# yeyupiaoling/VoiceprintRecognition-Pytorch

Measured on NVIDIA H100. Metric: embeddings/sec (3s@16kHz) ECAPA-TDNN, higher is better.
Workload: dtype f32

## Files before the change

voiceprintrecognition-pytorch_b200/csrc/api.cu:

```cuda
#include <cmath>
#include <cstdarg>
#include <cstdio>
#include <cstdlib>
#include <cstring>
#include <new>
#include <string>
#include <vector>

#include "kernels.cuh"


using namespace vpb;

struct vp_handle {
  int device = 0;
  std::string err;
  float* d_weights = nullptr;
  size_t weights_bytes = 0;
  char* d_arena = nullptr;
  size_t arena_bytes = 0;
  cudaStream_t cap_stream = nullptr;
  bool fe_set = false;
  vp_frontend_desc fe{};
  vp_frontend_options fe_opt{VP_FRAME_DEFAULT, 0, 1.0};
  float* d_window = nullptr;
  double2* d_twiddle = nullptr;
  int* d_mel_start = nullptr;
  int* d_mel_count = nullptr;
  int* d_mel_off = nullptr;
  float* d_mel_w = nullptr;
  float* d_dct = nullptr;
};

struct vp_program {
  vp_handle* h = nullptr;
  std::vector<vp_op> ops;
  std::vector<int> engines;
  size_t ws_bytes = 0, in_floats = 0, out_floats = 0;
  int launches = 0;
  int B = 0;
  cudaGraphExec_t gexec = nullptr;
  const float* g_feats = nullptr;
  float* g_emb = nullptr;
  char* g_arena = nullptr;
  int runs = 0, g_miss = 0;
  bool g_off = false;
  int n_slots = 0;
  size_t arena_need() const { return ws_bytes + (((size_t)n_slots * 4 + 255) & ~(size_t)255); }
  unsigned* slot(int32_t q) const { return q > 0 ? reinterpret_cast<unsigned*>(h->d_arena + ws_bytes) + (q - 1) : nullptr; }
};

static int fail(vp_handle* h, int code, const char* fmt, ...) {
  char buf[512];
  va_list ap;
  va_start(ap, fmt);
  vsnprintf(buf, sizeof(buf), fmt, ap);
  va_end(ap);
  if (h) h->err = buf;
  return code;
}
#define CUDA_TRY(h, expr)                                                                          \
  do {                                                                                             \
    cudaError_t e__ = (expr);                                                                      \
    if (e__ != cudaSuccess) return fail(h, VP_ERR_CUDA, "%s: %s", #expr, cudaGetErrorString(e__)); \
  } while (0)

static const int FPB = 16;

static bool tc16_enabled() {
  static int on = -1;
  if (on < 0) { const char* e = getenv("VPB_TC_F16"); on = (e && e[0] == '0') ? 0 : 1; }
  return on == 1;
}

extern "C" {

static void fill_conv(const vp_program* p, const vp_op& o, const float* feats, float* emb, vpb::ConvParams& c);

int vp_abi_version(void) { return VP_ABI_VERSION; }
int32_t vp_sizeof_op(void) { return (int32_t)sizeof(vp_op); }
int32_t vp_sizeof_frontend_desc(void) { return (int32_t)sizeof(vp_frontend_desc); }
int32_t vp_sizeof_frontend_options(void) { return (int32_t)sizeof(vp_frontend_options); }

int vp_create(int device, vp_handle** out) {
  if (!out) return VP_ERR_INVALID;
  *out = nullptr;
  int n = 0;
  cudaError_t e = cudaGetDeviceCount(&n);
  if (e != cudaSuccess || device < 0 || device >= n) return VP_ERR_CUDA;
  cudaDeviceProp prop;
  if (cudaGetDeviceProperties(&prop, device) != cudaSuccess) return VP_ERR_CUDA;
  if (prop.major != 9 || prop.minor != 0) return VP_ERR_UNSUPPORTED;
  if (cudaSetDevice(device) != cudaSuccess) return VP_ERR_CUDA;
  vp_handle* h = new (std::nothrow) vp_handle();
  if (!h) return VP_ERR_NOMEM;
  h->device = device;
  *out = h;
  return VP_OK;
}

// ... 405 lines not shown
    ConvParams c;
    fill_conv(p, o, nullptr, nullptr, c);
    c.amax_in = o.amax_in > 0 ? reinterpret_cast<const unsigned*>(8) : nullptr;
    const bool ok = conv_tc_supported(c);
    bool ok16 = ok && o.w_tc16_q > 0 && o.tc16_descale > 0.f && conv_tc16_supported(c);
    if (ok16) {
      const int bn = o.tc_bn, nt = (o.Cout + bn - 1) / bn, kb = (c.K + 63) / 64;
      const size_t off = (size_t)(o.w_tc16_q - 1) << 4, bytes = (size_t)nt * kb * 2 * bn * 128;
      if (off + bytes > h->weights_bytes) {
        int r = fail(h, VP_ERR_INVALID, "op %d: fp16 weight image out of range", i);
        delete p;
        return r;
      }
    }
    if ((o.engine == VP_ENGINE_TC && !ok) || (o.engine == VP_ENGINE_TC16 && !ok16)) {
      int r = fail(h, VP_ERR_UNSUPPORTED, "op %d: shape / operands not supported by the requested tensor-core engine", i);
      delete p;
      return r;
    }
    if (o.engine == VP_ENGINE_TC16 || (o.engine == VP_ENGINE_AUTO && ok16 && tc16_enabled())) p->engines[i] = VP_ENGINE_TC16;
    else if (o.engine == VP_ENGINE_TC || (o.engine == VP_ENGINE_AUTO && ok)) p->engines[i] = VP_ENGINE_TC;
    else p->engines[i] = VP_ENGINE_FFMA;
  }
  if (cudaSetDevice(h->device) != cudaSuccess) { delete p; return fail(h, VP_ERR_CUDA, "cudaSetDevice"); }
  if (p->arena_need() > h->arena_bytes) {
    const size_t want = p->arena_need() + (p->arena_need() >> 3);
    cudaDeviceSynchronize();
    cudaFree(h->d_arena);
    h->d_arena = nullptr;
    h->arena_bytes = 0;
    if (cudaMalloc(&h->d_arena, want) != cudaSuccess) {
      cudaGetLastError();
      if (cudaMalloc(&h->d_arena, p->arena_need()) != cudaSuccess) {
        delete p;
        return fail(h, VP_ERR_NOMEM, "workspace of %zu bytes: %s", ws_bytes, cudaGetErrorString(cudaGetLastError()));
      }
      h->arena_bytes = p->arena_need();
    } else {
      h->arena_bytes = want;
    }
  }
  *out = p;
  return VP_OK;
}

void vp_program_destroy(vp_program* p) {
// ... 18 lines not shown

static void fill_conv(const vp_program* p, const vp_op& o, const float* feats, float* emb, ConvParams& c) {
  c.src = rd(p, o.src, feats, emb);
  c.src2 = o.src2_mode == VP_SRC2_NONE ? nullptr : rd(p, o.src2, feats, emb);
  c.dst = const_cast<float*>(rd(p, o.dst, feats, emb));
  c.sum = const_cast<float*>(rd(p, o.sum, feats, emb)); c.sum_ld = o.sum_ld; c.sum_coff = o.sum_coff;
  c.res = rd(p, o.res, feats, emb); c.gate = rd(p, o.gate, feats, emb); c.ubias = rd(p, o.ubias, feats, emb);
  c.w = wt(p, o.w); c.w_tc = wt(p, o.w_tc); c.tc_bn = o.tc_bn; c.tc_kc = o.tc_kc; c.bias = wt(p, o.bias); c.pre_s = wt(p, o.pre_s); c.pre_h = wt(p, o.pre_h);
  c.post_s = wt(p, o.post_s); c.post_h = wt(p, o.post_h);
  c.B = o.B; c.Tin = o.Tin; c.Fin = o.Fin; c.Cin = o.Cin;
  c.CinTot = o.Cin + (o.src2_mode == VP_SRC2_CONCAT ? o.Cin2 : 0);
  c.in_ld = o.in_ld; c.in_coff = o.in_coff;
  c.src2_mode = o.src2_mode; c.src2_ld = o.src2_ld; c.src2_coff = o.src2_coff;
  c.Tout = o.Tout; c.Fout = o.Fout; c.out_ld = o.out_ld; c.out_coff = o.out_coff;
  c.res_ld = o.res_ld; c.res_coff = o.res_coff;
  c.KT = o.KT; c.KF = o.KF; c.sT = o.sT; c.sF = o.sF; c.dT = o.dT; c.dF = o.dF; c.padT = o.padT; c.padF = o.padF;
  c.pad_mode = o.pad_mode; c.w_ld = o.w_ld; c.pre_relu = o.pre_relu; c.act = o.act; c.act2 = o.act2;
  c.seg_len = o.seg_len; c.n_seg = o.n_seg;
  c.M = o.B * o.Tout * o.Fout; c.N = o.Cout; c.K = o.KT * o.KF * c.CinTot;
  c.amax_out = p->h->d_arena ? p->slot(o.amax_out) : nullptr;
  c.amax_in = p->h->d_arena ? p->slot(o.amax_in) : nullptr;
}

static int run_ops(vp_program* p, const float* feats, float* emb, cudaStream_t st, cudaEvent_t* evs) {
  vp_handle* h = p->h;
  if (p->n_slots > 0) CUDA_TRY(h, cudaMemsetAsync(h->d_arena + p->ws_bytes, 0, (size_t)p->n_slots * 4, st));
  for (size_t i = 0; i < p->ops.size(); ++i) {
    const vp_op& o = p->ops[i];
    if (evs) CUDA_TRY(h, cudaEventRecord(evs[i], st));
    switch (o.kind) {
      case VP_OP_CONV:
      case VP_OP_CONV_C1: {
        ConvParams c;
        fill_conv(p, o, feats, emb, c);
        if (o.kind == VP_OP_CONV_C1) {
          CUDA_TRY(h, launch_conv_c1(c, st));
        } else {
          if (p->engines[i] == VP_ENGINE_TC16)
            CUDA_TRY(h, launch_conv_tc16(c, reinterpret_cast<const float*>(reinterpret_cast<const char*>(h->d_weights) + ((size_t)(o.w_tc16_q - 1) << 4)),
                                         o.tc16_descale, st));
          else if (p->engines[i] == VP_ENGINE_TC) CUDA_TRY(h, launch_conv_tc(c, st));
          else CUDA_TRY(h, launch_conv_ffma(c, st));
        }
        break;
      }
      case VP_OP_COLSTATS: {
        StatsParams s;
        s.src = rd(p, o.src, feats, emb); s.dst = const_cast<float*>(rd(p, o.dst, feats, emb));
        s.B = o.B; s.R = o.Tin * o.Fin; s.C = o.Cin; s.in_ld = o.in_ld; s.in_coff = o.in_coff;
        s.out_ld = o.out_ld; s.out_coff = o.out_coff; s.mode = o.mode; s.seg_len = o.seg_len; s.n_seg = o.n_seg;
        s.eps = o.eps;
        CUDA_TRY(h, launch_colstats(s, st));
        break;
      }
      case VP_OP_ASP_POOL: {
        AspParams a;
        a.x = rd(p, o.src, feats, emb); a.logit = rd(p, o.src2, feats, emb);
        a.dst = const_cast<float*>(rd(p, o.dst, feats, emb));
        a.B = o.B; a.T = o.Tin; a.C = o.Cin; a.x_ld = o.in_ld; a.x_coff = o.in_coff; a.l_ld = o.src2_ld;
        a.l_coff = o.src2_coff; a.out_ld = o.out_ld; a.out_coff = o.out_coff; a.eps = o.eps; a.mean_only = o.mode == 1;
        CUDA_TRY(h, launch_asp_pool(a, st));
        break;
      }
      case VP_OP_POOL2D: {
        PoolParams q;
        q.src = rd(p, o.src, feats, emb); q.dst = const_cast<float*>(rd(p, o.dst, feats, emb));
        q.B = o.B; q.Tin = o.Tin; q.Fin = o.Fin; q.Tout = o.Tout; q.Fout = o.Fout; q.C = o.Cin;
        q.in_ld = o.in_ld; q.in_coff = o.in_coff; q.out_ld = o.out_ld; q.out_coff = o.out_coff;
        q.KT = o.KT; q.KF = o.KF; q.sT = o.sT; q.sF = o.sF; q.padT = o.padT; q.padF = o.padF; q.mode = o.mode;
        q.amax_out = p->slot(o.amax_out);
        CUDA_TRY(h, launch_pool2d(q, st));
        break;
      }
      case VP_OP_EW: {
        EwParams e;
        e.x = rd(p, o.src, feats, emb);
        e.y = o.mode == VP_EW_AFF ? rd(p, o.src2, feats, emb) : nullptr;
        e.att = o.mode == VP_EW_AFF ? rd(p, o.res, feats, emb) : nullptr;
        e.gate = o.mode == VP_EW_GATE_RES ? rd(p, o.gate, feats, emb) : nullptr;
        e.res = o.mode == VP_EW_GATE_RES ? rd(p, o.res, feats, emb) : nullptr;
        e.dst = const_cast<float*>(rd(p, o.dst, feats, emb));
        e.rows = (long long)o.B * o.Tin * o.Fin; e.C = o.Cin; e.rows_per_utt = o.Tin * o.Fin;
        e.x_ld = o.in_ld; e.x_coff = o.in_coff; e.y_ld = o.src2_ld; e.y_coff = o.src2_coff;
        e.att_ld = o.res_ld; e.att_coff = o.res_coff; e.res_ld = o.res_ld; e.res_coff = o.res_coff;
// ... 223 lines not shown
```

voiceprintrecognition-pytorch_b200/csrc/conv_tc.cu:

```cuda
#include <cuda_fp16.h>

#include <cstdlib>
#include <type_traits>

#include "kernels.cuh"
#include "wgmma.cuh"

namespace vpb {

namespace tc {

constexpr int BM = 128;
constexpr int BK = 32;
constexpr int A_TILE = BM * BK * 4;
constexpr int CONSUMER_WARPS = 8;
constexpr int CONSUMER_THREADS = CONSUMER_WARPS * 32;
constexpr int PRODUCER_WARPS = 8;
constexpr int PRODUCER_THREADS = PRODUCER_WARPS * 32;
constexpr int NUM_THREADS = CONSUMER_THREADS + PRODUCER_THREADS;
constexpr int ROWS_PER_THREAD = BM * 8 / PRODUCER_THREADS;
constexpr int MAX_BN = 128;
constexpr int MAX_BN_CHUNKED = 64;
constexpr int SMEM_BUDGET = 225 * 1024;

__device__ __forceinline__ uint32_t smem_u32(const void* p) { return (uint32_t)__cvta_generic_to_shared(p); }

__device__ __forceinline__ void mbar_init(uint32_t bar, uint32_t count) {
  asm volatile("mbarrier.init.shared::cta.b64 [%0], %1;" ::"r"(bar), "r"(count));
}
__device__ __forceinline__ void mbar_arrive(uint32_t bar) {
  asm volatile("mbarrier.arrive.shared::cta.b64 _, [%0];" ::"r"(bar) : "memory");
}
__device__ __forceinline__ void mbar_expect_tx(uint32_t bar, uint32_t bytes) {
  asm volatile("mbarrier.arrive.expect_tx.shared::cta.b64 _, [%0], %1;" ::"r"(bar), "r"(bytes) : "memory");
}
__device__ __forceinline__ void mbar_wait(uint32_t bar, uint32_t parity) {
  asm volatile(
      "{\n\t.reg .pred p;\n\t"
      "WAIT_%=:\n\t"
      "mbarrier.try_wait.parity.shared::cta.b64 p, [%0], %1;\n\t"
      "@p bra DONE_%=;\n\t"
      "bra WAIT_%=;\n\t"
      "DONE_%=:\n\t}" ::"r"(bar), "r"(parity)
      : "memory");
}
__device__ __forceinline__ void bulk_copy_g2s(uint32_t dst, const void* src, uint32_t bytes, uint32_t bar) {
  asm volatile("cp.async.bulk.shared::cluster.global.mbarrier::complete_tx::bytes [%0], [%1], %2, [%3];" ::"r"(dst),
               "l"(src), "r"(bytes), "r"(bar)
               : "memory");
}
__device__ __forceinline__ void fence_proxy_async() { asm volatile("fence.proxy.async.shared::cta;" ::: "memory"); }

__device__ __forceinline__ void wgmma_fence() { asm volatile("wgmma.fence.sync.aligned;" ::: "memory"); }
__device__ __forceinline__ void wgmma_commit() { asm volatile("wgmma.commit_group.sync.aligned;" ::: "memory"); }
template <int N>
__device__ __forceinline__ void wgmma_wait() { asm volatile("wgmma.wait_group.sync.aligned %0;" ::"n"(N) : "memory"); }
template <int N>
__device__ __forceinline__ void fence_regs(float (&d)[N]) {
#pragma unroll
  for (int i = 0; i < N; ++i) asm volatile("" : "+f"(d[i])::"memory");
}

__device__ __forceinline__ uint64_t smem_desc(uint32_t addr) {
  return (uint64_t)((addr >> 4) & 0x3FFF) | (1ull << 16) | (64ull << 32) | (1ull << 62);
}
__device__ __forceinline__ float tf32_rna(float x) {
  uint32_t r;
  asm("cvt.rna.tf32.f32 %0, %1;" : "=r"(r) : "f"(x));
  return __uint_as_float(r);
}

template <int BN, bool F16>
__device__ __forceinline__ void mma_tile(float* d, uint32_t a, uint32_t b, uint32_t scale_d) {
  const uint64_t da = smem_desc(a);
  if constexpr (BN == 128) {
    if constexpr (F16) wgmma_f16_n128(d, da, smem_desc(b), scale_d);
    else wgmma_tf32_n128(d, da, smem_desc(b), scale_d);
  } else {
    constexpr int o64 = 0, o32 = o64 + (BN & 64), o16 = o32 + (BN & 32);
    if constexpr ((BN & 64) != 0) {
      if constexpr (F16) wgmma_f16_n64(d + o64 / 2, da, smem_desc(b + o64 * 128), scale_d);
      else wgmma_tf32_n64(d + o64 / 2, da, smem_desc(b + o64 * 128), scale_d);
    }
    if constexpr ((BN & 32) != 0) {
      if constexpr (F16) wgmma_f16_n32(d + o32 / 2, da, smem_desc(b + o32 * 128), scale_d);
      else wgmma_tf32_n32(d + o32 / 2, da, smem_desc(b + o32 * 128), scale_d);
    }
    if constexpr ((BN & 16) != 0) {
      if constexpr (F16) wgmma_f16_n16(d + o16 / 2, da, smem_desc(b + o16 * 128), scale_d);
      else wgmma_tf32_n16(d + o16 / 2, da, smem_desc(b + o16 * 128), scale_d);
    }
  }
}

__device__ __noinline__ float2 act2_slow(float2 v, int act) {
  v.x = apply_act(v.x, act); v.y = apply_act(v.y, act);
  return v;
}

template <int MODE> struct Slot;
template <> struct Slot<0> { float4 v[ROWS_PER_THREAD]; };
template <> struct Slot<1> { float4 v[ROWS_PER_THREAD]; float4 u[ROWS_PER_THREAD]; };
template <> struct Slot<2> { float4 v[ROWS_PER_THREAD]; float4 ps, ph; uint32_t okmask; };
struct SlotH { float4 v[ROWS_PER_THREAD]; float4 w[ROWS_PER_THREAD]; };

struct TcArgs {
  const float* w_tc;
  int BN;
  int stages;
  int m_tiles, n_tiles, k_blocks;
  int kc, n_chunks;
  int debug;
  float descale;
};

// ... 116 lines not shown
      auto publish = [&](int q, SlotT& sl) {
        const int s = p_s;
        const uint32_t ph = p_ph;
        if (++p_s == S) { p_s = 0; p_ph ^= 1u; }
        mbar_wait(empty0 + 8 * s, ph ^ 1);
        if (t == 0) {
          if (a.debug & 1) {
            mbar_arrive(full0 + 8 * s);
          } else {
            const int tl = q / a.k_blocks, kb = q - tl * a.k_blocks;
            const int nt = ((int)blockIdx.x + tl * (int)gridDim.x) % a.n_tiles;
            const uint8_t* src = reinterpret_cast<const uint8_t*>(a.w_tc) + ((size_t)nt * a.k_blocks + kb) * (2u * b_tile);
            mbar_expect_tx(full0 + 8 * s, 2u * b_tile);
            bulk_copy_g2s(smem_base + s * stage_bytes + 2u * A_TILE, src, 2u * b_tile, full0 + 8 * s);
          }
        }
        const uint32_t a_hi = smem_base + s * stage_bytes;
        const uint32_t a_lo = a_hi + A_TILE;
#pragma unroll
        for (int i = 0; i < ROWS_PER_THREAD; ++i) {
          const int r = r0 + 32 * i;
          const uint32_t off = (uint32_t)r * 128u + (uint32_t)((chunk ^ (r & 7)) << 4);
          if constexpr (F16) {
            const float xs[8] = {sl.v[i].x * ascale, sl.v[i].y * ascale, sl.v[i].z * ascale, sl.v[i].w * ascale,
                                 sl.w[i].x * ascale, sl.w[i].y * ascale, sl.w[i].z * ascale, sl.w[i].w * ascale};
            uint32_t hw[4], lw[4];
#pragma unroll
            for (int j = 0; j < 4; ++j) {
              const __half2 h = __floats2half2_rn(xs[2 * j], xs[2 * j + 1]);
              const float2 hf = __half22float2(h);
              const __half2 l = __floats2half2_rn(xs[2 * j] - hf.x, xs[2 * j + 1] - hf.y);
              hw[j] = *reinterpret_cast<const uint32_t*>(&h);
              lw[j] = *reinterpret_cast<const uint32_t*>(&l);
            }
            asm volatile("st.shared.v4.b32 [%0], {%1, %2, %3, %4};" ::"r"(a_hi + off), "r"(hw[0]), "r"(hw[1]), "r"(hw[2]), "r"(hw[3]) : "memory");
            asm volatile("st.shared.v4.b32 [%0], {%1, %2, %3, %4};" ::"r"(a_lo + off), "r"(lw[0]), "r"(lw[1]), "r"(lw[2]), "r"(lw[3]) : "memory");
            continue;
          }
          float4 x = sl.v[i];
          if constexpr (MODE == 1) { x.x += sl.u[i].x; x.y += sl.u[i].y; x.z += sl.u[i].z; x.w += sl.u[i].w; }
          if constexpr (MODE == 2) {
            if (sl.okmask & (1u << i)) {
              x.x = fmaf(x.x, sl.ps.x, sl.ph.x); x.y = fmaf(x.y, sl.ps.y, sl.ph.y);
              x.z = fmaf(x.z, sl.ps.z, sl.ph.z); x.w = fmaf(x.w, sl.ps.w, sl.ph.w);
              if (p.pre_relu) { x.x = fmaxf(x.x, 0.f); x.y = fmaxf(x.y, 0.f); x.z = fmaxf(x.z, 0.f); x.w = fmaxf(x.w, 0.f); }
            }
          }
          float4 hi, lo;
          hi.x = tf32_rna(x.x); hi.y = tf32_rna(x.y); hi.z = tf32_rna(x.z); hi.w = tf32_rna(x.w);
          lo.x = x.x - hi.x; lo.y = x.y - hi.y; lo.z = x.z - hi.z; lo.w = x.w - hi.w;
          asm volatile("st.shared.v4.f32 [%0], {%1, %2, %3, %4};" ::"r"(a_hi + off), "f"(hi.x), "f"(hi.y), "f"(hi.z), "f"(hi.w) : "memory");
          asm volatile("st.shared.v4.f32 [%0], {%1, %2, %3, %4};" ::"r"(a_lo + off), "f"(lo.x), "f"(lo.y), "f"(lo.z), "f"(lo.w) : "memory");
        }
        fence_proxy_async();
        __syncwarp();
        if (lane == 0) mbar_arrive(full0 + 8 * s);
        if (q + DEPTH < total_items) gather(sl);
// ... 286 lines not shown
```

voiceprintrecognition-pytorch_b200/csrc/kernels.cuh:

```cuda
#pragma once
#include "common.cuh"

namespace vpb {

struct FrontendParams {
  const float* wave; float* feats; float* partial;
  const float* window; const double2* twiddle;
  const int* mel_start; const int* mel_count; const int* mel_off; const float* mel_w;
  int B, L, T, kind, N, WL, hop, F, remove_dc, power, use_log, fpb, nblk;
  int frame;
  int pad;
  double spec_mult;
  float preemph, log_floor, db_mult;
  float* cta_max;
  int n_pass, radix[12], G;
};
void frontend_plan(FrontendParams& p);

struct MfccParams {
  const float* mel; const float* cta_max; const float* dct; float* feats; float* partial;
  int B, T, M, K, fpb, nblk, n_max;
  float top_db;
};

// ... 40 lines not shown
                                uint8_t* sorted_labels, vp_verify_result* result, cudaStream_t stream);

cudaError_t launch_resample(const float* x, int64_t in_ld, float* y, int64_t out_ld, int B, const int64_t* n_in,
                            const int64_t* n_out, const int32_t* up, const int32_t* down, const int64_t* tap_off,
                            const double* taps, cudaStream_t stream);
size_t gain_scratch_bytes(int B, int64_t ld);
cudaError_t launch_gain(float* w, int64_t ld, int B, const int64_t* lens, double target_db, double max_gain_db,
                        int32_t* flags, void* scratch, cudaStream_t stream);

cudaError_t launch_frontend(const FrontendParams& p, const int* keep, cudaStream_t stream);
cudaError_t launch_frontend_mfcc(const FrontendParams& p, const MfccParams& m, const int* keep, cudaStream_t stream);
cudaError_t launch_frontend_mfcc_mel(const FrontendParams& p, float* max_out, cudaStream_t stream);
cudaError_t launch_frontend_mfcc_finish(const FrontendParams& p, const MfccParams& m, const int* keep, cudaStream_t stream);
size_t frontend_smem_bytes(int N, int WL, int hop, int fpb);
cudaError_t launch_conv_ffma(const ConvParams& p, cudaStream_t stream);
cudaError_t launch_conv_c1(const ConvParams& p, cudaStream_t stream);
cudaError_t launch_colstats(const StatsParams& p, cudaStream_t stream);
cudaError_t launch_asp_pool(const AspParams& p, cudaStream_t stream);
cudaError_t launch_ew(const EwParams& p, cudaStream_t stream);
bool conv_tc_supported(const ConvParams& p);
cudaError_t launch_conv_tc(const ConvParams& p, cudaStream_t stream);
bool conv_tc16_supported(const ConvParams& p);
cudaError_t launch_conv_tc16(const ConvParams& p, const float* w_tc16, float descale, cudaStream_t stream);

}
```

voiceprintrecognition-pytorch_b200/csrc/wgmma.cuh:

```cuda
#pragma once
#include <stdint.h>

namespace vpb {
namespace tc {

__device__ __forceinline__ void wgmma_tf32_n16(float* d, uint64_t a, uint64_t b, uint32_t scale_d) {
  asm volatile(
      "{\n\t.reg .pred p;\n\tsetp.ne.b32 p, %10, 0;\n\t"
      "wgmma.mma_async.sync.aligned.m64n16k8.f32.tf32.tf32 {%0, %1, %2, %3, %4, %5, %6, %7}, %8, %9, p, 1, 1;\n\t}"
      : "+f"(d[0]), "+f"(d[1]), "+f"(d[2]), "+f"(d[3]), "+f"(d[4]), "+f"(d[5]), "+f"(d[6]), "+f"(d[7])
      : "l"(a), "l"(b), "r"(scale_d));
}
__device__ __forceinline__ void wgmma_tf32_n32(float* d, uint64_t a, uint64_t b, uint32_t scale_d) {
  asm volatile(
      "{\n\t.reg .pred p;\n\tsetp.ne.b32 p, %18, 0;\n\t"
      "wgmma.mma_async.sync.aligned.m64n32k8.f32.tf32.tf32 {%0, %1, %2, %3, %4, %5, %6, %7, %8, %9, %10, %11, %12, %13, %14, %15}, %16, %17, p, 1, 1;\n\t}"
      : "+f"(d[0]), "+f"(d[1]), "+f"(d[2]), "+f"(d[3]), "+f"(d[4]), "+f"(d[5]), "+f"(d[6]), "+f"(d[7]), "+f"(d[8]), "+f"(d[9]), "+f"(d[10]), "+f"(d[11]), "+f"(d[12]), "+f"(d[13]), "+f"(d[14]), "+f"(d[15])
      : "l"(a), "l"(b), "r"(scale_d));
}
__device__ __forceinline__ void wgmma_tf32_n64(float* d, uint64_t a, uint64_t b, uint32_t scale_d) {
  asm volatile(
      "{\n\t.reg .pred p;\n\tsetp.ne.b32 p, %34, 0;\n\t"
      "wgmma.mma_async.sync.aligned.m64n64k8.f32.tf32.tf32 {%0, %1, %2, %3, %4, %5, %6, %7, %8, %9, %10, %11, %12, %13, %14, %15, %16, %17, %18, %19, %20, %21, %22, %23, %24, %25, %26, %27, %28, %29, %30, %31}, %32, %33, p, 1, 1;\n\t}"
      : "+f"(d[0]), "+f"(d[1]), "+f"(d[2]), "+f"(d[3]), "+f"(d[4]), "+f"(d[5]), "+f"(d[6]), "+f"(d[7]), "+f"(d[8]), "+f"(d[9]), "+f"(d[10]), "+f"(d[11]), "+f"(d[12]), "+f"(d[13]), "+f"(d[14]), "+f"(d[15]), "+f"(d[16]), "+f"(d[17]), "+f"(d[18]), "+f"(d[19]), "+f"(d[20]), "+f"(d[21]), "+f"(d[22]), "+f"(d[23]), "+f"(d[24]), "+f"(d[25]), "+f"(d[26]), "+f"(d[27]), "+f"(d[28]), "+f"(d[29]), "+f"(d[30]), "+f"(d[31])
// ... 15 lines not shown
}
__device__ __forceinline__ void wgmma_f16_n32(float* d, uint64_t a, uint64_t b, uint32_t scale_d) {
  asm volatile(
      "{\n\t.reg .pred p;\n\tsetp.ne.b32 p, %18, 0;\n\t"
      "wgmma.mma_async.sync.aligned.m64n32k16.f32.f16.f16 {%0, %1, %2, %3, %4, %5, %6, %7, %8, %9, %10, %11, %12, %13, %14, %15}, %16, %17, p, 1, 1, 0, 0;\n\t}"
      : "+f"(d[0]), "+f"(d[1]), "+f"(d[2]), "+f"(d[3]), "+f"(d[4]), "+f"(d[5]), "+f"(d[6]), "+f"(d[7]), "+f"(d[8]), "+f"(d[9]), "+f"(d[10]), "+f"(d[11]), "+f"(d[12]), "+f"(d[13]), "+f"(d[14]), "+f"(d[15])
      : "l"(a), "l"(b), "r"(scale_d));
}
__device__ __forceinline__ void wgmma_f16_n64(float* d, uint64_t a, uint64_t b, uint32_t scale_d) {
  asm volatile(
      "{\n\t.reg .pred p;\n\tsetp.ne.b32 p, %34, 0;\n\t"
      "wgmma.mma_async.sync.aligned.m64n64k16.f32.f16.f16 {%0, %1, %2, %3, %4, %5, %6, %7, %8, %9, %10, %11, %12, %13, %14, %15, %16, %17, %18, %19, %20, %21, %22, %23, %24, %25, %26, %27, %28, %29, %30, %31}, %32, %33, p, 1, 1, 0, 0;\n\t}"
      : "+f"(d[0]), "+f"(d[1]), "+f"(d[2]), "+f"(d[3]), "+f"(d[4]), "+f"(d[5]), "+f"(d[6]), "+f"(d[7]), "+f"(d[8]), "+f"(d[9]), "+f"(d[10]), "+f"(d[11]), "+f"(d[12]), "+f"(d[13]), "+f"(d[14]), "+f"(d[15]), "+f"(d[16]), "+f"(d[17]), "+f"(d[18]), "+f"(d[19]), "+f"(d[20]), "+f"(d[21]), "+f"(d[22]), "+f"(d[23]), "+f"(d[24]), "+f"(d[25]), "+f"(d[26]), "+f"(d[27]), "+f"(d[28]), "+f"(d[29]), "+f"(d[30]), "+f"(d[31])
      : "l"(a), "l"(b), "r"(scale_d));
}
__device__ __forceinline__ void wgmma_f16_n128(float* d, uint64_t a, uint64_t b, uint32_t scale_d) {
  asm volatile(
      "{\n\t.reg .pred p;\n\tsetp.ne.b32 p, %66, 0;\n\t"
      "wgmma.mma_async.sync.aligned.m64n128k16.f32.f16.f16 {%0, %1, %2, %3, %4, %5, %6, %7, %8, %9, %10, %11, %12, %13, %14, %15, %16, %17, %18, %19, %20, %21, %22, %23, %24, %25, %26, %27, %28, %29, %30, %31, %32, %33, %34, %35, %36, %37, %38, %39, %40, %41, %42, %43, %44, %45, %46, %47, %48, %49, %50, %51, %52, %53, %54, %55, %56, %57, %58, %59, %60, %61, %62, %63}, %64, %65, p, 1, 1, 0, 0;\n\t}"
      : "+f"(d[0]), "+f"(d[1]), "+f"(d[2]), "+f"(d[3]), "+f"(d[4]), "+f"(d[5]), "+f"(d[6]), "+f"(d[7]), "+f"(d[8]), "+f"(d[9]), "+f"(d[10]), "+f"(d[11]), "+f"(d[12]), "+f"(d[13]), "+f"(d[14]), "+f"(d[15]), "+f"(d[16]), "+f"(d[17]), "+f"(d[18]), "+f"(d[19]), "+f"(d[20]), "+f"(d[21]), "+f"(d[22]), "+f"(d[23]), "+f"(d[24]), "+f"(d[25]), "+f"(d[26]), "+f"(d[27]), "+f"(d[28]), "+f"(d[29]), "+f"(d[30]), "+f"(d[31]), "+f"(d[32]), "+f"(d[33]), "+f"(d[34]), "+f"(d[35]), "+f"(d[36]), "+f"(d[37]), "+f"(d[38]), "+f"(d[39]), "+f"(d[40]), "+f"(d[41]), "+f"(d[42]), "+f"(d[43]), "+f"(d[44]), "+f"(d[45]), "+f"(d[46]), "+f"(d[47]), "+f"(d[48]), "+f"(d[49]), "+f"(d[50]), "+f"(d[51]), "+f"(d[52]), "+f"(d[53]), "+f"(d[54]), "+f"(d[55]), "+f"(d[56]), "+f"(d[57]), "+f"(d[58]), "+f"(d[59]), "+f"(d[60]), "+f"(d[61]), "+f"(d[62]), "+f"(d[63])
      : "l"(a), "l"(b), "r"(scale_d));
}

}
}
```

Before: 29240.

## Fuse attention logit 1x1 conv into attentive statistics pooling kernel

Adds a fused kernel that computes the final attention-logit 1x1 convolution with fp16 split-precision wgmma directly into a shared-memory strip, then performs the softmax-weighted mean/std pooling in the same block. The planner detects eligible conv+ASP pairs, checks that the logits buffer is not read elsewhere, and skips the separate conv launch. This removes one kernel launch and the global write and re-read of the logits tensor. In exchange the grid is only channel-tiles × batch with one large-smem block each, which may underuse the GPU compared with the separate kernels.

```diff
diff --git a/voiceprintrecognition-pytorch_b200/csrc/api.cu b/voiceprintrecognition-pytorch_b200/csrc/api.cu
--- a/voiceprintrecognition-pytorch_b200/csrc/api.cu
+++ b/voiceprintrecognition-pytorch_b200/csrc/api.cu
@@ -36,6 +36,7 @@
   vp_handle* h = nullptr;
   std::vector<vp_op> ops;
   std::vector<int> engines;
+  std::vector<char> fused;
   size_t ws_bytes = 0, in_floats = 0, out_floats = 0;
   int launches = 0;
   int B = 0;
@@ -76,6 +77,8 @@
 extern "C" {
 
 static void fill_conv(const vp_program* p, const vp_op& o, const float* feats, float* emb, vpb::ConvParams& c);
+static void fill_asp(const vp_program* p, const vp_op& o, const float* feats, float* emb, vpb::AspParams& a);
+static void mark_fused_heads(vp_program* p);
 
 int vp_abi_version(void) { return VP_ABI_VERSION; }
 int32_t vp_sizeof_op(void) { return (int32_t)sizeof(vp_op); }
@@ -527,6 +530,7 @@
     else if (o.engine == VP_ENGINE_TC || (o.engine == VP_ENGINE_AUTO && ok)) p->engines[i] = VP_ENGINE_TC;
     else p->engines[i] = VP_ENGINE_FFMA;
   }
+  mark_fused_heads(p);
   if (cudaSetDevice(h->device) != cudaSuccess) { delete p; return fail(h, VP_ERR_CUDA, "cudaSetDevice"); }
   if (p->arena_need() > h->arena_bytes) {
     const size_t want = p->arena_need() + (p->arena_need() >> 3);
@@ -591,6 +595,80 @@
   c.amax_in = p->h->d_arena ? p->slot(o.amax_in) : nullptr;
 }
 
+static void fill_asp(const vp_program* p, const vp_op& o, const float* feats, float* emb, AspParams& a) {
+  a.x = rd(p, o.src, feats, emb); a.logit = rd(p, o.src2, feats, emb);
+  a.dst = const_cast<float*>(rd(p, o.dst, feats, emb));
+  a.B = o.B; a.T = o.Tin; a.C = o.Cin; a.x_ld = o.in_ld; a.x_coff = o.in_coff; a.l_ld = o.src2_ld;
+  a.l_coff = o.src2_coff; a.out_ld = o.out_ld; a.out_coff = o.out_coff; a.eps = o.eps; a.mean_only = o.mode == 1;
+}
+
+struct ByteRange { int64_t lo = 0, hi = 0; };
+static ByteRange ws_range(int64_t off, long long rows, int ld) {
+  ByteRange r;
+  if (off < 0 || rows < 1) return r;
+  r.lo = off; r.hi = off + (int64_t)rows * ld * 4;
+  return r;
+}
+static bool overlaps(ByteRange a, ByteRange b) { return a.lo < a.hi && b.lo < b.hi && a.lo < b.hi && b.lo < a.hi; }
+
+static std::vector<ByteRange> op_reads(const vp_op& o) {
+  std::vector<ByteRange> r;
+  const long long rows_in = (long long)o.B * o.Tin * o.Fin, rows_out = (long long)o.B * o.Tout * o.Fout;
+  r.push_back(ws_range(o.src, rows_in, o.in_ld));
+  switch (o.kind) {
+    case VP_OP_CONV:
+    case VP_OP_CONV_C1:
+      if (o.src2_mode != VP_SRC2_NONE) r.push_back(ws_range(o.src2, rows_in, o.src2_ld));
+      r.push_back(ws_range(o.res, rows_out, o.res_ld));
+      r.push_back(ws_range(o.sum, rows_out, o.sum_ld));
+      r.push_back(ws_range(o.gate, (long long)o.B * o.n_seg, o.Cout));
+      r.push_back(ws_range(o.ubias, (long long)o.B * o.n_seg, o.Cout));
+      break;
+    case VP_OP_ASP_POOL:
+      r.push_back(ws_range(o.src2, rows_in, o.src2_ld));
+      break;
+    case VP_OP_EW:
+      r.push_back(ws_range(o.src2, rows_in, o.src2_ld));
+      r.push_back(ws_range(o.res, rows_in, o.res_ld));
+      r.push_back(ws_range(o.gate, o.B, o.Cin));
+      break;
+    default:
+      break;
+  }
+  return r;
+}
+
+static void mark_fused_heads(vp_program* p) {
+  const int n = (int)p->ops.size();
+  p->fused.assign(n, 0);
+  for (int i = 0; i + 1 < n; ++i) {
+    const vp_op& o = p->ops[i];
+    const vp_op& q = p->ops[i + 1];
+    if (o.kind != VP_OP_CONV || p->engines[i] != VP_ENGINE_TC16 || q.kind != VP_OP_ASP_POOL) continue;
+    if (o.dst < 0 || q.src2 != o.dst || q.src2_ld != o.out_ld || q.src2_coff != o.out_coff || q.Cin != o.Cout) continue;
+    ConvParams c;
+    fill_conv(p, o, nullptr, nullptr, c);
+    c.amax_in = o.amax_in > 0 ? reinterpret_cast<const unsigned*>(8) : nullptr;
+    c.amax_out = o.amax_out > 0 ? reinterpret_cast<unsigned*>(8) : nullptr;
+    const float* some = reinterpret_cast<const float*>(8);
+    c.res = o.res != VP_BUF_NONE ? some : nullptr; c.gate = o.gate != VP_BUF_NONE ? some : nullptr;
+    c.ubias = o.ubias != VP_BUF_NONE ? some : nullptr; c.sum = o.sum != VP_BUF_NONE ? const_cast<float*>(some) : nullptr;
+    AspParams a;
+    fill_asp(p, q, nullptr, nullptr, a);
+    if (!asp_fused_supported(c, a)) continue;
+    const ByteRange logits = ws_range(o.dst, (long long)o.B * o.Tout, o.out_ld);
+    bool read_elsewhere = overlaps(logits, ws_range(o.src, (long long)o.B * o.Tin, o.in_ld)) ||
+                          overlaps(logits, ws_range(q.src, (long long)q.B * q.Tin, q.in_ld));
+    for (int j = i + 2; j < n && !read_elsewhere; ++j)
+      for (const ByteRange& r : op_reads(p->ops[j]))
+        if (overlaps(logits, r)) { read_elsewhere = true; break; }
+    if (read_elsewhere) continue;
+    p->fused[i] = p->fused[i + 1] = 1;
+    --p->launches;
+    ++i;
+  }
+}
+
 static int run_ops(vp_program* p, const float* feats, float* emb, cudaStream_t st, cudaEvent_t* evs) {
   vp_handle* h = p->h;
   if (p->n_slots > 0) CUDA_TRY(h, cudaMemsetAsync(h->d_arena + p->ws_bytes, 0, (size_t)p->n_slots * 4, st));
@@ -600,6 +678,7 @@
     switch (o.kind) {
       case VP_OP_CONV:
       case VP_OP_CONV_C1: {
+        if (p->fused[i]) break;
         ConvParams c;
         fill_conv(p, o, feats, emb, c);
         if (o.kind == VP_OP_CONV_C1) {
@@ -624,11 +703,17 @@
       }
       case VP_OP_ASP_POOL: {
         AspParams a;
-        a.x = rd(p, o.src, feats, emb); a.logit = rd(p, o.src2, feats, emb);
-        a.dst = const_cast<float*>(rd(p, o.dst, feats, emb));
-        a.B = o.B; a.T = o.Tin; a.C = o.Cin; a.x_ld = o.in_ld; a.x_coff = o.in_coff; a.l_ld = o.src2_ld;
-        a.l_coff = o.src2_coff; a.out_ld = o.out_ld; a.out_coff = o.out_coff; a.eps = o.eps; a.mean_only = o.mode == 1;
-        CUDA_TRY(h, launch_asp_pool(a, st));
+        fill_asp(p, o, feats, emb, a);
+        if (p->fused[i]) {
+          const vp_op& lo = p->ops[i - 1];
+          ConvParams c;
+          fill_conv(p, lo, feats, emb, c);
+          CUDA_TRY(h, launch_asp_fused(c, a, reinterpret_cast<const float*>(reinterpret_cast<const char*>(h->d_weights) +
+                                                                            ((size_t)(lo.w_tc16_q - 1) << 4)),
+                                       lo.tc16_descale, st));
+        } else {
+          CUDA_TRY(h, launch_asp_pool(a, st));
+        }
         break;
       }
       case VP_OP_POOL2D: {
diff --git a/voiceprintrecognition-pytorch_b200/csrc/asp_fused.cu b/voiceprintrecognition-pytorch_b200/csrc/asp_fused.cu
--- /dev/null
+++ b/voiceprintrecognition-pytorch_b200/csrc/asp_fused.cu
@@ -0,0 +1,272 @@
+#include "kernels.cuh"
+#include "wgmma.cuh"
+
+namespace vpb {
+
+namespace {
+
+constexpr int AF_THREADS = 256;
+constexpr int AF_BN = 128;
+constexpr int AF_ROWS = 64;
+constexpr int AF_KB_MAX = 2;
+constexpr int AF_SMEM_MAX = 226 * 1024;
+constexpr int AF_T_MIN = 128;
+constexpr int AF_XU = 8;
+
+struct AspFusedArgs {
+  const float* w_img;
+  float descale;
+  int Tp;
+};
+
+__device__ __forceinline__ int strip_idx(int row, int col) { return row * AF_BN + (col ^ ((row & 7) << 3)); }
+
+__device__ __forceinline__ float4 block_reduce4(float4 v, bool is_max, float* red, float* bc) {
+  const int lane = threadIdx.x & 31, wid = threadIdx.x >> 5;
+  reinterpret_cast<float4*>(red)[wid * 32 + lane] = v;
+  __syncthreads();
+  if (wid == 0) {
+    float4 s = reinterpret_cast<const float4*>(red)[lane];
+#pragma unroll
+    for (int i = 1; i < 8; ++i) {
+      const float4 r = reinterpret_cast<const float4*>(red)[i * 32 + lane];
+      if (is_max) { s.x = fmaxf(s.x, r.x); s.y = fmaxf(s.y, r.y); s.z = fmaxf(s.z, r.z); s.w = fmaxf(s.w, r.w); }
+      else { s.x = s.x + r.x; s.y = s.y + r.y; s.z = s.z + r.z; s.w = s.w + r.w; }
+    }
+    reinterpret_cast<float4*>(bc)[lane] = s;
+  }
+  __syncthreads();
+  const float4 r = reinterpret_cast<const float4*>(bc)[lane];
+  __syncthreads();
+  return r;
+}
+
+__device__ __forceinline__ void wg_sync(int wg) {
+  asm volatile("bar.sync %0, 128;" ::"r"(wg + 1) : "memory");
+}
+
+template <int KB>
+__global__ void __launch_bounds__(AF_THREADS, 1) asp_fused_kernel(const __grid_constant__ ConvParams c,
+                                                                 const __grid_constant__ AspParams a,
+                                                                 const __grid_constant__ AspFusedArgs f) {
+  using namespace tc;
+  pdl_launch_dependents();
+  extern __shared__ uint8_t smem_raw[];
+  __shared__ __align__(8) uint64_t wbar;
+  const uint32_t base = (smem_u32(smem_raw) + 1023u) & ~1023u;
+  uint8_t* const gbase = smem_raw + (base - smem_u32(smem_raw));
+  const uint32_t strip_s = base + (uint32_t)KB * 32768u;
+  float* const strip = reinterpret_cast<float*>(gbase + (size_t)KB * 32768u);
+  const int warp = threadIdx.x >> 5, lane = threadIdx.x & 31;
+  const int nb = blockIdx.x, b = blockIdx.y;
+  const int n0 = nb * AF_BN;
+  const int T = a.T;
+
+  const uint32_t bar = smem_u32(&wbar);
+  if (threadIdx.x == 0) {
+    mbar_init(bar, 1);
+    asm volatile("fence.mbarrier_init.release.cluster;" ::: "memory");
+    mbar_expect_tx(bar, (uint32_t)KB * 32768u);
+    const uint8_t* src = reinterpret_cast<const uint8_t*>(f.w_img) + (size_t)nb * KB * 32768u;
+    for (int kb = 0; kb < KB; ++kb) bulk_copy_g2s(base + kb * 32768u, src + kb * 32768u, 32768u, bar);
+  }
+  __syncthreads();
+  pdl_wait();
+
+  {
+    const float* xb = a.x + (size_t)b * T * a.x_ld + a.x_coff + n0;
+    const int ncols = min(AF_BN, a.C - n0);
+    for (int i = threadIdx.x; i < T * 4; i += AF_THREADS) {
+      const int t = i >> 2, seg = (i & 3) * 32;
+      if (seg < ncols) asm volatile("prefetch.global.L2 [%0];" ::"l"(xb + (size_t)t * a.x_ld + seg));
+    }
+  }
+
+  {
+    const int wg = warp >> 2, t = threadIdx.x & 127;
+    const int chunk = t & 7, r0 = t >> 3;
+    const float ascale = exp2i(f16_scale_exp(__ldg(c.amax_in)));
+    const float descale = f.descale * exp2i(-f16_scale_exp(__ldg(c.amax_in)));
+    const int q4 = lane & 3;
+    const int rfrag = 16 * (warp & 3) + (lane >> 2);
+    const float* hb = c.src + (size_t)b * T * c.in_ld + c.in_coff;
+    float acc[AF_BN / 2];
+#pragma unroll
+    for (int i = 0; i < AF_BN / 2; ++i) acc[i] = 0.f;
+    bool first_tile = true;
+    for (int rt = wg; rt * AF_ROWS < f.Tp; rt += 2) {
+      const uint32_t a_s = strip_s + (uint32_t)rt * (AF_ROWS * AF_BN * 4);
+#pragma unroll
+      for (int kb = 0; kb < KB; ++kb) {
+        const int k = kb * 64 + chunk * 8;
+        float4 v[4], w[4];
+#pragma unroll
+        for (int i = 0; i < 4; ++i) {
+          const int row = rt * AF_ROWS + r0 + 16 * i;
+          v[i] = make_float4(0.f, 0.f, 0.f, 0.f);
+          w[i] = v[i];
+          if (row < T && k < c.K) {
+            const float4* g = reinterpret_cast<const float4*>(hb + (size_t)row * c.in_ld + k);
+            v[i] = __ldg(g);
+            w[i] = __ldg(g + 1);
+          }
+        }
+#pragma unroll
+        for (int i = 0; i < 4; ++i) {
+          const int r = r0 + 16 * i;
+          const uint32_t off = (uint32_t)r * 128u + (uint32_t)((chunk ^ (r & 7)) << 4);
+          const uint32_t a_hi = a_s + kb * 16384u, a_lo = a_hi + 8192u;
+          uint32_t hw[4], lw[4];
+          split_f16x8(v[i], w[i], ascale, hw, lw);
+          asm volatile("st.shared.v4.b32 [%0], {%1, %2, %3, %4};" ::"r"(a_hi + off), "r"(hw[0]), "r"(hw[1]), "r"(hw[2]), "r"(hw[3]) : "memory");
+          asm volatile("st.shared.v4.b32 [%0], {%1, %2, %3, %4};" ::"r"(a_lo + off), "r"(lw[0]), "r"(lw[1]), "r"(lw[2]), "r"(lw[3]) : "memory");
+        }
+      }
+      fence_proxy_async();
+      wg_sync(wg);
+      if (first_tile) { mbar_wait(bar, 0); first_tile = false; }
+      wgmma_fence();
+#pragma unroll
+      for (int kb = 0; kb < KB; ++kb) {
+        const uint32_t a_hi = a_s + kb * 16384u, a_lo = a_hi + 8192u;
+        const uint32_t b_hi = base + kb * 32768u, b_lo = b_hi + 16384u;
+#pragma unroll
+        for (int kk = 0; kk < 4; ++kk) {
+          mma_tile<AF_BN, true>(acc, a_lo + kk * 32, b_hi + kk * 32, (kb != 0) || (kk != 0));
+          mma_tile<AF_BN, true>(acc, a_hi + kk * 32, b_lo + kk * 32, 1);
+          mma_tile<AF_BN, true>(acc, a_hi + kk * 32, b_hi + kk * 32, 1);
+        }
+      }
+      wgmma_commit();
+      wgmma_wait<0>();
+      fence_regs(acc);
+      wg_sync(wg);
+#pragma unroll
+      for (int j = 0; j < AF_BN / 8; ++j) {
+        const int n = n0 + 8 * j + 2 * q4;
+        float2 b2 = make_float2(0.f, 0.f);
+        if (c.bias && n < c.N) b2 = __ldg(reinterpret_cast<const float2*>(c.bias + n));
+#pragma unroll
+        for (int h = 0; h < 2; ++h) {
+          const int row = rt * AF_ROWS + rfrag + 8 * h;
+          float2 x = make_float2(acc[4 * j + 2 * h], acc[4 * j + 2 * h + 1]);
+          x.x = fmaf(x.x, descale, b2.x); x.y = fmaf(x.y, descale, b2.y);
+          *reinterpret_cast<float2*>(strip + strip_idx(row, 8 * j + 2 * q4)) = x;
+        }
+      }
+    }
+  }
+  __syncthreads();
+
+  float* red = reinterpret_cast<float*>(gbase);
+  float* bc = red + 8 * AF_BN;
+  const int col = 4 * lane;
+  const int cg = n0 + col;
+  const bool ok = cg < a.C;
+  const float* xb = a.x + (size_t)b * T * a.x_ld + a.x_coff + cg;
+  auto xrow = [&](int t) {
+    return ok ? __ldg(reinterpret_cast<const float4*>(xb + (size_t)t * a.x_ld)) : make_float4(0.f, 0.f, 0.f, 0.f);
+  };
+  auto srow = [&](int t) -> float4& { return *reinterpret_cast<float4*>(strip + strip_idx(t, col)); };
+
+  float4 mx = make_float4(-INFINITY, -INFINITY, -INFINITY, -INFINITY);
+  for (int t = warp; t < T; t += 8) {
+    const float4 l = srow(t);
+    mx.x = fmaxf(mx.x, l.x); mx.y = fmaxf(mx.y, l.y); mx.z = fmaxf(mx.z, l.z); mx.w = fmaxf(mx.w, l.w);
+  }
+  mx = block_reduce4(mx, true, red, bc);
+  float4 se = make_float4(0.f, 0.f, 0.f, 0.f), sxe = se;
+  for (int t0 = warp; t0 < T; t0 += 8 * AF_XU) {
+    float4 xv[AF_XU];
+#pragma unroll
+    for (int u = 0; u < AF_XU; ++u) if (t0 + 8 * u < T) xv[u] = xrow(t0 + 8 * u);
+#pragma unroll
+    for (int u = 0; u < AF_XU; ++u) {
+      const int t = t0 + 8 * u;
+      if (t >= T) break;
+      float4& l = srow(t);
+      float4 e;
+      e.x = expf(l.x - mx.x); e.y = expf(l.y - mx.y); e.z = expf(l.z - mx.z); e.w = expf(l.w - mx.w);
+      l = e;
+      se.x += e.x; se.y += e.y; se.z += e.z; se.w += e.w;
+      sxe.x = fmaf(e.x, xv[u].x, sxe.x); sxe.y = fmaf(e.y, xv[u].y, sxe.y);
+      sxe.z = fmaf(e.z, xv[u].z, sxe.z); sxe.w = fmaf(e.w, xv[u].w, sxe.w);
+    }
+  }
+  se = block_reduce4(se, false, red, bc);
+  sxe = block_reduce4(sxe, false, red, bc);
+  const float4 mean = make_float4(sxe.x / se.x, sxe.y / se.y, sxe.z / se.z, sxe.w / se.w);
+  float4 sq = make_float4(0.f, 0.f, 0.f, 0.f);
+  if (!a.mean_only) {
+    for (int t0 = warp; t0 < T; t0 += 8 * AF_XU) {
+      float4 xv[AF_XU];
+#pragma unroll
+      for (int u = 0; u < AF_XU; ++u) if (t0 + 8 * u < T) xv[u] = xrow(t0 + 8 * u);
+#pragma unroll
+      for (int u = 0; u < AF_XU; ++u) {
+        const int t = t0 + 8 * u;
+        if (t >= T) break;
+        const float4 e = srow(t);
+        const float dx = xv[u].x - mean.x, dy = xv[u].y - mean.y, dz = xv[u].z - mean.z, dw = xv[u].w - mean.w;
+        sq.x = fmaf(e.x, dx * dx, sq.x); sq.y = fmaf(e.y, dy * dy, sq.y);
+        sq.z = fmaf(e.z, dz * dz, sq.z); sq.w = fmaf(e.w, dw * dw, sq.w);
+      }
+    }
+    sq = block_reduce4(sq, false, red, bc);
+  }
+  if (warp == 0 && ok) {
+    float* o = a.dst + (size_t)b * a.out_ld + a.out_coff;
+    o[cg] = mean.x; o[cg + 1] = mean.y; o[cg + 2] = mean.z; o[cg + 3] = mean.w;
+    if (!a.mean_only) {
+      o[a.C + cg] = sqrtf(fmaxf(sq.x / se.x, a.eps));
+      o[a.C + cg + 1] = sqrtf(fmaxf(sq.y / se.y, a.eps));
+      o[a.C + cg + 2] = sqrtf(fmaxf(sq.z / se.z, a.eps));
+      o[a.C + cg + 3] = sqrtf(fmaxf(sq.w / se.w, a.eps));
+    }
+  }
+}
+
+size_t asp_fused_smem(int T, int K) {
+  const int Tp = (T + AF_ROWS - 1) / AF_ROWS * AF_ROWS;
+  const int kb = (K + 63) / 64;
+  return 1024 + (size_t)kb * 32768 + (size_t)Tp * AF_BN * 4;
+}
+
+}
+
+bool asp_fused_supported(const ConvParams& c, const AspParams& a) {
+  if (c.KT != 1 || c.KF != 1 || c.Fin != 1 || c.Fout != 1 || c.sT != 1 || c.padT != 0) return false;
+  if (c.src2_mode != VP_SRC2_NONE || c.pre_s || c.post_s || c.res || c.gate || c.ubias || c.sum) return false;
+  if (c.act != VP_ACT_NONE || c.act2 != VP_ACT_NONE || c.amax_out || !c.amax_in) return false;
+  if (c.tc_bn != AF_BN || (c.tc_kc > 0 && c.tc_kc < c.K) || c.K > AF_KB_MAX * 64 || (c.K & 7)) return false;
+  if (c.B != a.B || c.Tin != a.T || c.Tout != a.T || c.N != a.C || a.T < AF_T_MIN) return false;
+  if ((a.C & 3) || (a.x_ld & 3) || (a.x_coff & 3)) return false;
+  return asp_fused_smem(a.T, c.K) <= (size_t)AF_SMEM_MAX;
+}
+
+template <int KB>
+static cudaError_t launch_kb(dim3 grid, size_t smem, cudaStream_t stream, const ConvParams& c, const AspParams& a,
+                             const AspFusedArgs& f) {
+  static PerDeviceSmem once;
+  if (once.need(smem)) {
+    cudaError_t e = cudaFuncSetAttribute(asp_fused_kernel<KB>, cudaFuncAttributeMaxDynamicSharedMemorySize, AF_SMEM_MAX);
+    if (e != cudaSuccess) return e;
+    once.set(AF_SMEM_MAX);
+  }
+  launch_pdl(asp_fused_kernel<KB>, grid, dim3(AF_THREADS), smem, stream, c, a, f);
+  return cudaGetLastError();
+}
+
+cudaError_t launch_asp_fused(const ConvParams& c, const AspParams& a, const float* w_tc16, float descale,
+                             cudaStream_t stream) {
+  AspFusedArgs f;
+  f.w_img = w_tc16;
+  f.descale = descale;
+  f.Tp = (a.T + AF_ROWS - 1) / AF_ROWS * AF_ROWS;
+  const size_t smem = asp_fused_smem(a.T, c.K);
+  const dim3 grid((a.C + AF_BN - 1) / AF_BN, a.B);
+  if (c.K > 64) return launch_kb<2>(grid, smem, stream, c, a, f);
+  return launch_kb<1>(grid, smem, stream, c, a, f);
+}
+
+}
diff --git a/voiceprintrecognition-pytorch_b200/csrc/conv_tc.cu b/voiceprintrecognition-pytorch_b200/csrc/conv_tc.cu
--- a/voiceprintrecognition-pytorch_b200/csrc/conv_tc.cu
+++ b/voiceprintrecognition-pytorch_b200/csrc/conv_tc.cu
@@ -23,74 +23,10 @@
 constexpr int MAX_BN_CHUNKED = 64;
 constexpr int SMEM_BUDGET = 225 * 1024;
 
-__device__ __forceinline__ uint32_t smem_u32(const void* p) { return (uint32_t)__cvta_generic_to_shared(p); }
-
-__device__ __forceinline__ void mbar_init(uint32_t bar, uint32_t count) {
-  asm volatile("mbarrier.init.shared::cta.b64 [%0], %1;" ::"r"(bar), "r"(count));
-}
-__device__ __forceinline__ void mbar_arrive(uint32_t bar) {
-  asm volatile("mbarrier.arrive.shared::cta.b64 _, [%0];" ::"r"(bar) : "memory");
-}
-__device__ __forceinline__ void mbar_expect_tx(uint32_t bar, uint32_t bytes) {
-  asm volatile("mbarrier.arrive.expect_tx.shared::cta.b64 _, [%0], %1;" ::"r"(bar), "r"(bytes) : "memory");
-}
-__device__ __forceinline__ void mbar_wait(uint32_t bar, uint32_t parity) {
-  asm volatile(
-      "{\n\t.reg .pred p;\n\t"
-      "WAIT_%=:\n\t"
-      "mbarrier.try_wait.parity.shared::cta.b64 p, [%0], %1;\n\t"
-      "@p bra DONE_%=;\n\t"
-      "bra WAIT_%=;\n\t"
-      "DONE_%=:\n\t}" ::"r"(bar), "r"(parity)
-      : "memory");
-}
-__device__ __forceinline__ void bulk_copy_g2s(uint32_t dst, const void* src, uint32_t bytes, uint32_t bar) {
-  asm volatile("cp.async.bulk.shared::cluster.global.mbarrier::complete_tx::bytes [%0], [%1], %2, [%3];" ::"r"(dst),
-               "l"(src), "r"(bytes), "r"(bar)
-               : "memory");
-}
-__device__ __forceinline__ void fence_proxy_async() { asm volatile("fence.proxy.async.shared::cta;" ::: "memory"); }
-
-__device__ __forceinline__ void wgmma_fence() { asm volatile("wgmma.fence.sync.aligned;" ::: "memory"); }
-__device__ __forceinline__ void wgmma_commit() { asm volatile("wgmma.commit_group.sync.aligned;" ::: "memory"); }
-template <int N>
-__device__ __forceinline__ void wgmma_wait() { asm volatile("wgmma.wait_group.sync.aligned %0;" ::"n"(N) : "memory"); }
-template <int N>
-__device__ __forceinline__ void fence_regs(float (&d)[N]) {
-#pragma unroll
-  for (int i = 0; i < N; ++i) asm volatile("" : "+f"(d[i])::"memory");
-}
-
-__device__ __forceinline__ uint64_t smem_desc(uint32_t addr) {
-  return (uint64_t)((addr >> 4) & 0x3FFF) | (1ull << 16) | (64ull << 32) | (1ull << 62);
-}
 __device__ __forceinline__ float tf32_rna(float x) {
   uint32_t r;
   asm("cvt.rna.tf32.f32 %0, %1;" : "=r"(r) : "f"(x));
   return __uint_as_float(r);
-}
-
-template <int BN, bool F16>
-__device__ __forceinline__ void mma_tile(float* d, uint32_t a, uint32_t b, uint32_t scale_d) {
-  const uint64_t da = smem_desc(a);
-  if constexpr (BN == 128) {
-    if constexpr (F16) wgmma_f16_n128(d, da, smem_desc(b), scale_d);
-    else wgmma_tf32_n128(d, da, smem_desc(b), scale_d);
-  } else {
-    constexpr int o64 = 0, o32 = o64 + (BN & 64), o16 = o32 + (BN & 32);
-    if constexpr ((BN & 64) != 0) {
-      if constexpr (F16) wgmma_f16_n64(d + o64 / 2, da, smem_desc(b + o64 * 128), scale_d);
-      else wgmma_tf32_n64(d + o64 / 2, da, smem_desc(b + o64 * 128), scale_d);
-    }
-    if constexpr ((BN & 32) != 0) {
-      if constexpr (F16) wgmma_f16_n32(d + o32 / 2, da, smem_desc(b + o32 * 128), scale_d);
-      else wgmma_tf32_n32(d + o32 / 2, da, smem_desc(b + o32 * 128), scale_d);
-    }
-    if constexpr ((BN & 16) != 0) {
-      if constexpr (F16) wgmma_f16_n16(d + o16 / 2, da, smem_desc(b + o16 * 128), scale_d);
-      else wgmma_tf32_n16(d + o16 / 2, da, smem_desc(b + o16 * 128), scale_d);
-    }
-  }
 }
 
 __device__ __noinline__ float2 act2_slow(float2 v, int act) {
@@ -253,17 +189,8 @@
           const int r = r0 + 32 * i;
           const uint32_t off = (uint32_t)r * 128u + (uint32_t)((chunk ^ (r & 7)) << 4);
           if constexpr (F16) {
-            const float xs[8] = {sl.v[i].x * ascale, sl.v[i].y * ascale, sl.v[i].z * ascale, sl.v[i].w * ascale,
-                                 sl.w[i].x * ascale, sl.w[i].y * ascale, sl.w[i].z * ascale, sl.w[i].w * ascale};
             uint32_t hw[4], lw[4];
-#pragma unroll
-            for (int j = 0; j < 4; ++j) {
-              const __half2 h = __floats2half2_rn(xs[2 * j], xs[2 * j + 1]);
-              const float2 hf = __half22float2(h);
-              const __half2 l = __floats2half2_rn(xs[2 * j] - hf.x, xs[2 * j + 1] - hf.y);
-              hw[j] = *reinterpret_cast<const uint32_t*>(&h);
-              lw[j] = *reinterpret_cast<const uint32_t*>(&l);
-            }
+            split_f16x8(sl.v[i], sl.w[i], ascale, hw, lw);
             asm volatile("st.shared.v4.b32 [%0], {%1, %2, %3, %4};" ::"r"(a_hi + off), "r"(hw[0]), "r"(hw[1]), "r"(hw[2]), "r"(hw[3]) : "memory");
             asm volatile("st.shared.v4.b32 [%0], {%1, %2, %3, %4};" ::"r"(a_lo + off), "r"(lw[0]), "r"(lw[1]), "r"(lw[2]), "r"(lw[3]) : "memory");
             continue;
diff --git a/voiceprintrecognition-pytorch_b200/csrc/kernels.cuh b/voiceprintrecognition-pytorch_b200/csrc/kernels.cuh
--- a/voiceprintrecognition-pytorch_b200/csrc/kernels.cuh
+++ b/voiceprintrecognition-pytorch_b200/csrc/kernels.cuh
@@ -86,5 +86,7 @@
 cudaError_t launch_conv_tc(const ConvParams& p, cudaStream_t stream);
 bool conv_tc16_supported(const ConvParams& p);
 cudaError_t launch_conv_tc16(const ConvParams& p, const float* w_tc16, float descale, cudaStream_t stream);
+bool asp_fused_supported(const ConvParams& c, const AspParams& a);
+cudaError_t launch_asp_fused(const ConvParams& c, const AspParams& a, const float* w_tc16, float descale, cudaStream_t stream);
 
 }
diff --git a/voiceprintrecognition-pytorch_b200/csrc/wgmma.cuh b/voiceprintrecognition-pytorch_b200/csrc/wgmma.cuh
--- a/voiceprintrecognition-pytorch_b200/csrc/wgmma.cuh
+++ b/voiceprintrecognition-pytorch_b200/csrc/wgmma.cuh
@@ -1,4 +1,5 @@
 #pragma once
+#include <cuda_fp16.h>
 #include <stdint.h>
 
 namespace vpb {
@@ -61,5 +62,84 @@
       : "l"(a), "l"(b), "r"(scale_d));
 }
 
+
+__device__ __forceinline__ uint32_t smem_u32(const void* p) { return (uint32_t)__cvta_generic_to_shared(p); }
+
+__device__ __forceinline__ void mbar_init(uint32_t bar, uint32_t count) {
+  asm volatile("mbarrier.init.shared::cta.b64 [%0], %1;" ::"r"(bar), "r"(count));
+}
+__device__ __forceinline__ void mbar_arrive(uint32_t bar) {
+  asm volatile("mbarrier.arrive.shared::cta.b64 _, [%0];" ::"r"(bar) : "memory");
+}
+__device__ __forceinline__ void mbar_expect_tx(uint32_t bar, uint32_t bytes) {
+  asm volatile("mbarrier.arrive.expect_tx.shared::cta.b64 _, [%0], %1;" ::"r"(bar), "r"(bytes) : "memory");
+}
+__device__ __forceinline__ void mbar_wait(uint32_t bar, uint32_t parity) {
+  asm volatile(
+      "{\n\t.reg .pred p;\n\t"
+      "WAIT_%=:\n\t"
+      "mbarrier.try_wait.parity.shared::cta.b64 p, [%0], %1;\n\t"
+      "@p bra DONE_%=;\n\t"
+      "bra WAIT_%=;\n\t"
+      "DONE_%=:\n\t}" ::"r"(bar), "r"(parity)
+      : "memory");
+}
+__device__ __forceinline__ void bulk_copy_g2s(uint32_t dst, const void* src, uint32_t bytes, uint32_t bar) {
+  asm volatile("cp.async.bulk.shared::cluster.global.mbarrier::complete_tx::bytes [%0], [%1], %2, [%3];" ::"r"(dst),
+               "l"(src), "r"(bytes), "r"(bar)
+               : "memory");
+}
+__device__ __forceinline__ void fence_proxy_async() { asm volatile("fence.proxy.async.shared::cta;" ::: "memory"); }
+
+__device__ __forceinline__ void wgmma_fence() { asm volatile("wgmma.fence.sync.aligned;" ::: "memory"); }
+__device__ __forceinline__ void wgmma_commit() { asm volatile("wgmma.commit_group.sync.aligned;" ::: "memory"); }
+template <int N>
+__device__ __forceinline__ void wgmma_wait() { asm volatile("wgmma.wait_group.sync.aligned %0;" ::"n"(N) : "memory"); }
+template <int N>
+__device__ __forceinline__ void fence_regs(float (&d)[N]) {
+#pragma unroll
+  for (int i = 0; i < N; ++i) asm volatile("" : "+f"(d[i])::"memory");
+}
+
+__device__ __forceinline__ uint64_t smem_desc(uint32_t addr) {
+  return (uint64_t)((addr >> 4) & 0x3FFF) | (1ull << 16) | (64ull << 32) | (1ull << 62);
+}
+template <int BN, bool F16>
+__device__ __forceinline__ void mma_tile(float* d, uint32_t a, uint32_t b, uint32_t scale_d) {
+  const uint64_t da = smem_desc(a);
+  if constexpr (BN == 128) {
+    if constexpr (F16) wgmma_f16_n128(d, da, smem_desc(b), scale_d);
+    else wgmma_tf32_n128(d, da, smem_desc(b), scale_d);
+  } else {
+    constexpr int o64 = 0, o32 = o64 + (BN & 64), o16 = o32 + (BN & 32);
+    if constexpr ((BN & 64) != 0) {
+      if constexpr (F16) wgmma_f16_n64(d + o64 / 2, da, smem_desc(b + o64 * 128), scale_d);
+      else wgmma_tf32_n64(d + o64 / 2, da, smem_desc(b + o64 * 128), scale_d);
+    }
+    if constexpr ((BN & 32) != 0) {
+      if constexpr (F16) wgmma_f16_n32(d + o32 / 2, da, smem_desc(b + o32 * 128), scale_d);
+      else wgmma_tf32_n32(d + o32 / 2, da, smem_desc(b + o32 * 128), scale_d);
+    }
+    if constexpr ((BN & 16) != 0) {
+      if constexpr (F16) wgmma_f16_n16(d + o16 / 2, da, smem_desc(b + o16 * 128), scale_d);
+      else wgmma_tf32_n16(d + o16 / 2, da, smem_desc(b + o16 * 128), scale_d);
+    }
+  }
+}
+
+
+__device__ __forceinline__ void split_f16x8(const float4& v, const float4& w, float scale, uint32_t (&hw)[4],
+                                            uint32_t (&lw)[4]) {
+  const float xs[8] = {v.x * scale, v.y * scale, v.z * scale, v.w * scale, w.x * scale, w.y * scale, w.z * scale, w.w * scale};
+#pragma unroll
+  for (int j = 0; j < 4; ++j) {
+    const __half2 h = __floats2half2_rn(xs[2 * j], xs[2 * j + 1]);
+    const float2 hf = __half22float2(h);
+    const __half2 l = __floats2half2_rn(xs[2 * j] - hf.x, xs[2 * j + 1] - hf.y);
+    hw[j] = *reinterpret_cast<const uint32_t*>(&h);
+    lw[j] = *reinterpret_cast<const uint32_t*>(&l);
+  }
+}
+
 }
 }
```

New measurement: 29610, median of 6. 1.2% higher.
